# dordanino12/unet-convlstm

Measured on AMD Instinct MI355X. Metric: training frames/sec, Moving-MNIST 64x64 seq-20, higher is better.
Workload: dtype bf16; 1 GPU; TemporalUNetDualView(base_ch=64, use_skip_lstm=True) train step, 64x64 seq-20, per-GPU batch 32, AdamW+clip; global_batch=32, seq_len=20, parallelism=dp1

## Files before the change

### include/uclstm.h

```cpp
#ifndef UCLSTM_H
#define UCLSTM_H

#include <stdint.h>

#ifdef __cplusplus
extern "C" {
#endif

#define UCLSTM_ABI_VERSION 16

#define UCLSTM_OK            0
#define UCLSTM_E_BADARG     -1
#define UCLSTM_E_LAUNCH     -2
#define UCLSTM_E_NODEVICE   -3

#define UCLSTM_ACT_TYPE_BF16 0
#define UCLSTM_ACT_TYPE_F16  1


typedef struct {
    const void* ptr;
    int32_t C;
    int32_t Hs, Ws;
    int32_t offY, offX;
// ... 416 lines not shown
int32_t uclstm_head3x3_bwd_ordered(const void* a, const float* w, const float* dy, void* da, float* partials, float* dw, float* db,
                                   int32_t accumulate, int64_t n_img, int32_t H, int32_t W, int32_t Cp, int32_t C, int32_t Co,
                                   int32_t act_type, void* stream);

int32_t uclstm_maxpool3s2_bwd(const void* a, const void* dp, const void* dskip, void* da, int32_t n_img, int32_t H, int32_t W,
                              int32_t Cp, void* stream);
int64_t uclstm_bn_add_relu_bwd_rows(int64_t pixels);
int32_t uclstm_bn_add_relu_bwd_reduce(const void* z, const float* scale, const float* shift, const float* mean, const float* rstd,
                                      const void* r, const float* rscale, const float* rshift, const float* rmean,
                                      const float* rrstd, const void* da, float* partials, float* sums, float* rsums,
                                      int64_t pixels, int32_t Cp, void* stream);
int32_t uclstm_bn_add_relu_bwd_apply(const void* z, const float* scale, const float* shift, const float* mean, const float* rstd,
                                     const float* sums, const void* r, const float* rscale, const float* rshift,
                                     const float* rmean, const float* rrstd, const float* rsums, const void* da, void* dz,
                                     void* dr, int64_t pixels, int32_t Cp, void* stream);

#define UCLSTM_F16_TWIN(fn) __typeof__(fn) fn##_f16;
UCLSTM_F16_TWIN(uclstm_igemm_fwd)
UCLSTM_F16_TWIN(uclstm_igemm_fwd_group)
UCLSTM_F16_TWIN(uclstm_igemm_wgrad)
UCLSTM_F16_TWIN(uclstm_pack_weights)
UCLSTM_F16_TWIN(uclstm_pack_weights_batched)
UCLSTM_F16_TWIN(uclstm_bn_apply_relu)
UCLSTM_F16_TWIN(uclstm_bn_bwd_reduce)
UCLSTM_F16_TWIN(uclstm_bn_bwd_apply)
UCLSTM_F16_TWIN(uclstm_bn_apply_relu_pool)
UCLSTM_F16_TWIN(uclstm_bn_pool_bwd_reduce)
UCLSTM_F16_TWIN(uclstm_bn_pool_bwd_apply)
UCLSTM_F16_TWIN(uclstm_bn_head_fwd)
UCLSTM_F16_TWIN(uclstm_bn_head_bwd_reduce)
// ... 10 lines not shown
UCLSTM_F16_TWIN(uclstm_im2col3x3_first)
UCLSTM_F16_TWIN(uclstm_outconv_fwd)
UCLSTM_F16_TWIN(uclstm_outconv_bwd)
UCLSTM_F16_TWIN(uclstm_colsum)
UCLSTM_F16_TWIN(uclstm_attention_fwd)
UCLSTM_F16_TWIN(uclstm_attention_bwd)
#define UCLSTM_RESNET_F16_TWINS(TWIN) \
    TWIN(uclstm_im2col7x7s2_first) TWIN(uclstm_maxpool3s2_fwd) TWIN(uclstm_bn_add_relu) TWIN(uclstm_upsample2_fwd) \
    TWIN(uclstm_upsample2_bwd) TWIN(uclstm_head3x3_fwd) TWIN(uclstm_head3x3_bwd)
UCLSTM_RESNET_F16_TWINS(UCLSTM_F16_TWIN)
#define UCLSTM_RESNET_BWD_F16_TWINS(TWIN) \
    TWIN(uclstm_maxpool3s2_bwd) TWIN(uclstm_bn_add_relu_bwd_reduce) TWIN(uclstm_bn_add_relu_bwd_apply)
UCLSTM_RESNET_BWD_F16_TWINS(UCLSTM_F16_TWIN)
#define UCLSTM_TAP_GROUP_F16_TWINS(TWIN) TWIN(uclstm_igemm_fwd_group_tap)
UCLSTM_TAP_GROUP_F16_TWINS(UCLSTM_F16_TWIN)

int32_t uclstm_abi_version(void);
const char* uclstm_build_arch(void);
const char* uclstm_source_hash(void);
const char* uclstm_last_error_string(void);

#ifdef __cplusplus
}
#endif
#endif
```

### unet-convlstm_amd/_lib.py

```python
from __future__ import annotations

import ctypes as C
import os
import re

import torch

HERE = os.path.dirname(os.path.abspath(__file__))
LIB_PATH = os.environ.get("UCLSTM_LIB") or os.path.join(HERE, "libuclstm.so")
HEADER_PATH = os.path.join(HERE, "..", "include", "uclstm.h")

ABI_VERSION = 16
EPI_STORE, EPI_LSTM, EPI_ATOMIC = 0, 1, 2
NMODE_IDENTITY, NMODE_LSTM, NMODE_TAPMAJOR = 0, 1, 2
KMODE_IDENTITY, KMODE_GATES, KMODE_IM2COL = 0, 1, 2
ACT_TYPE_BF16, ACT_TYPE_F16 = 0, 1

_ERRORS = {-1: "bad argument (shape/alignment/null contract)", -2: "kernel launch failed", -3: "no gfx950 device"}


class UclstmError(RuntimeError):
    pass


# ... 82 lines not shown

class EvalVecDesc(C.Structure):
    _fields_ = [("y_pred", C.c_void_p), ("pred_stride_b", C.c_int64), ("pred_stride_t", C.c_int64),
                ("y", C.c_void_p), ("y_stride_b", C.c_int64), ("y_stride_t", C.c_int64),
                ("mask", C.c_void_p), ("mask_stride_b", C.c_int64), ("mask_stride_t", C.c_int64),
                ("B", C.c_int32), ("T", C.c_int32), ("Cy", C.c_int32), ("transform", C.c_int32), ("HW", C.c_int64),
                ("consts", TargetConsts * 4),
                ("hist_lo", C.c_double * 4), ("hist_hi", C.c_double * 4), ("err_lo", C.c_double * 4), ("err_hi", C.c_double * 4),
                ("dig_lo", C.c_double * 4), ("dig_w", C.c_double * 4),
                ("bins", C.c_int32), ("n_edges", C.c_int32), ("K", C.c_int32), ("dir_bins", C.c_int32),
                ("seed", C.c_uint64),
                ("w_chan", C.c_int32), ("h_chan", C.c_int32), ("w_sign", C.c_int32), ("h_sign", C.c_int32),
                ("speed_hi", C.c_double), ("epe_hi", C.c_double), ("min_speed", C.c_double),
                ("table", C.c_void_p), ("hist", C.c_void_p), ("dig_count", C.c_void_p), ("scatter", C.c_void_p),
                ("vtable", C.c_void_p), ("vhist", C.c_void_p), ("dir_hist", C.c_void_p)]


LOSS_POINT_L1, LOSS_POINT_L2, LOSS_POINT_HUBER = 0, 1, 2
VEC_MAX = 4
SELECT_MAX_SLOTS, SELECT_BINS, SELECT_SIGNED, SELECT_ABS = 8, 2048, 0, 1
SELECT_WS_COUNT, SELECT_WS_NAN, SELECT_WS_FLAGS, SELECT_WS_PREFIX, SELECT_WS_RANK, SELECT_WS_LEADER, SELECT_WS_HIST = 0, 1, 2, 8, 16, 24, 32
EXTREMES_MIN_KEY, EXTREMES_MAX_KEY, EXTREMES_NAN, EXTREMES_NONZERO, EXTREMES_COUNT, EXTREMES_WORDS = 0, 1, 2, 3, 4, 8
EVAL_ROW = 16
EVAL_VROW = 16
EVAL_NONE, EVAL_ASINH, EVAL_SIGNED_LOG = 0, 1, 2

_P, _I, _L, _F = C.c_void_p, C.c_int32, C.c_int64, C.c_float

_PROTOS = {
    "uclstm_igemm_tiles_per_group": [_I, _I, _I, _I, _I],
# ... 98 lines not shown
    "uclstm_metric_sums": [_P, _P, _P, _P, _L, _F, _F, _F, _P],
    "uclstm_metric_sums_ordered_rows": [_L],
    "uclstm_metric_sums_ordered": [_P, _P, _P, _P, _P, _I, _L, _F, _F, _F, _P],
    "uclstm_metric_sums_vec_rows": [_L, _I, _I],
    "uclstm_metric_sums_vec": [_P, _P, _P, _P, _P, _I, _L, _I, _I, _I, C.POINTER(TargetConsts), _P],
    "uclstm_eval_stats": [C.POINTER(EvalDesc), _P],
    "uclstm_eval_stats_rows": [_L, _L],
    "uclstm_eval_stats_vec": [C.POINTER(EvalVecDesc), _P],
    "uclstm_select_workspace_bytes": [],
    "uclstm_select_begin": [C.POINTER(SelectState), _P, C.POINTER(C.c_int64), C.POINTER(C.c_int32), _I, _P],
    "uclstm_select_accumulate": [C.POINTER(SelectState), _I, _P, _L, _P],
    "uclstm_select_narrow": [C.POINTER(SelectState), _I, _P],
    "uclstm_select_finish": [C.POINTER(SelectState), _P, _P, _P],
    "uclstm_dataset_extremes_begin": [_P, _P],
    "uclstm_dataset_extremes": [_P, _L, _P, _P],
    "uclstm_stream_spin": [_I, _P],
    "uclstm_abi_version": [],
    "uclstm_build_arch": [],
    "uclstm_source_hash": [],
    "uclstm_last_error_string": [],
}
_RESTYPES = {"uclstm_build_arch": C.c_char_p, "uclstm_source_hash": C.c_char_p, "uclstm_last_error_string": C.c_char_p, "uclstm_bn_bwd_reduce_rows": C.c_int64, "uclstm_bn_pool_bwd_rows": C.c_int64,
             "uclstm_eval_stats_rows": C.c_int64, "uclstm_colsum_ordered_rows": C.c_int64, "uclstm_outconv_bwd_ordered_rows": C.c_int64, "uclstm_head3x3_bwd_ordered_rows": C.c_int64,
             "uclstm_loss_fwd_ordered_rows": C.c_int64, "uclstm_sumsq_ordered_rows": C.c_int64, "uclstm_metric_sums_ordered_rows": C.c_int64, "uclstm_metric_sums_vec_rows": C.c_int64,
             "uclstm_bn_add_relu_bwd_rows": C.c_int64, "uclstm_select_workspace_bytes": C.c_int64}


F16_TWINS = ['uclstm_igemm_fwd', 'uclstm_igemm_fwd_group', 'uclstm_igemm_wgrad', 'uclstm_pack_weights', 'uclstm_pack_weights_batched', 'uclstm_bn_apply_relu', 'uclstm_bn_bwd_reduce', 'uclstm_bn_bwd_apply', 'uclstm_bn_apply_relu_pool', 'uclstm_bn_pool_bwd_reduce', 'uclstm_bn_pool_bwd_apply', 'uclstm_bn_head_fwd', 'uclstm_bn_head_bwd_reduce', 'uclstm_bn_head_bwd_apply', 'uclstm_maxpool2_fwd', 'uclstm_maxpool2_bwd', 'uclstm_lstm_bwd_pointwise', 'uclstm_lstm_fwd_pointwise', 'uclstm_lstm_fwd_pointwise_group', 'uclstm_splitk_finish', 'uclstm_nchw_to_nhwc', 'uclstm_nhwc_to_nchw', 'uclstm_nchw_grad_to_nhwc', 'uclstm_im2col3x3_first', 'uclstm_outconv_fwd', 'uclstm_outconv_bwd', 'uclstm_colsum', 'uclstm_attention_fwd', 'uclstm_attention_bwd']
RESNET_F16_TWINS = ['uclstm_im2col7x7s2_first', 'uclstm_maxpool3s2_fwd', 'uclstm_bn_add_relu', 'uclstm_upsample2_fwd', 'uclstm_upsample2_bwd',
                    'uclstm_head3x3_fwd', 'uclstm_head3x3_bwd']
RESNET_BWD_F16_TWINS = ['uclstm_maxpool3s2_bwd', 'uclstm_bn_add_relu_bwd_reduce', 'uclstm_bn_add_relu_bwd_apply']
TAP_GROUP_F16_TWINS = ['uclstm_igemm_fwd_group_tap']
_ALL_F16_TWINS = frozenset(F16_TWINS) | frozenset(RESNET_F16_TWINS) | frozenset(RESNET_BWD_F16_TWINS) | frozenset(TAP_GROUP_F16_TWINS)


def header_symbols() -> list[str]:
    with open(HEADER_PATH) as f:
        text = f.read()
    names = set(re.findall(r"\b(uclstm_[a-z0-9_]+)\s*\(", text))
    names |= {n + "_f16" for n in re.findall(r"^UCLSTM_F16_TWIN\((uclstm_[a-z0-9_]+)\)", text, re.M)}
    return sorted(names)


def _load() -> C.CDLL:
    if not os.path.exists(LIB_PATH):
        raise UclstmError(
            f"{LIB_PATH} is missing: build it with `python unet-convlstm_amd/build.py` "
            "(hipcc --offload-arch=gfx950). There is no CPU or PyTorch fallback for this package.")
# ... 55 lines not shown
```

### unet-convlstm_amd/build.py

```python
from __future__ import annotations

import hashlib
import os
import subprocess
import sys
from concurrent.futures import ThreadPoolExecutor

HERE = os.path.dirname(os.path.abspath(__file__))
CSRC = os.path.join(HERE, "csrc")
HEADER = os.path.join(HERE, "..", "include", "uclstm.h")
LIB = os.path.join(HERE, "libuclstm.so")
SOURCES = ["igemm_fwd.hip", "igemm_wgrad.hip", "pointwise.hip", "pack.hip", "loss_optim.hip", "eval_stats.hip", "augment.hip", "sprites.hip", "resnet.hip", "resnet_bwd.hip", "dataset_stats.hip"]
F16_SOURCES = ["igemm_fwd.hip", "igemm_wgrad.hip", "pointwise.hip", "pack.hip", "resnet.hip", "resnet_bwd.hip"]
FLAGS = ["--offload-arch=gfx950", "-O3", "-std=c++17", "-fPIC", "-fno-gpu-rdc", "-Wno-unused-result"]
F16_FLAGS = ["-DUCLSTM_ACT_F16", "-Wno-unused-function"]


def _hipcc() -> str:
    for c in (os.environ.get("HIPCC"), "/opt/rocm/bin/hipcc", "hipcc"):
        if c and (os.path.isabs(c) and os.path.exists(c) or not os.path.isabs(c)):
            return c
    raise RuntimeError("hipcc not found")


def _sha(parts) -> str:
    h = hashlib.sha256()
    for p in parts:
        if isinstance(p, str):
# ... 96 lines not shown
```

### unet-convlstm_amd/csrc/common.h

```cpp
#pragma once
#include <hip/hip_runtime.h>
#include <stdint.h>

#if defined(UCLSTM_ACT_F16)
#define uclstm_igemm_fwd uclstm_igemm_fwd_f16
#define uclstm_igemm_fwd_group uclstm_igemm_fwd_group_f16
#define uclstm_igemm_fwd_group_tap uclstm_igemm_fwd_group_tap_f16
#define uclstm_igemm_wgrad uclstm_igemm_wgrad_f16
#define uclstm_pack_weights uclstm_pack_weights_f16
#define uclstm_pack_weights_batched uclstm_pack_weights_batched_f16
#define uclstm_splitk_finish uclstm_splitk_finish_f16
#define uclstm_bn_apply_relu uclstm_bn_apply_relu_f16
#define uclstm_bn_bwd_reduce uclstm_bn_bwd_reduce_f16
#define uclstm_bn_bwd_apply uclstm_bn_bwd_apply_f16
#define uclstm_bn_head_fwd uclstm_bn_head_fwd_f16
#define uclstm_bn_apply_relu_pool uclstm_bn_apply_relu_pool_f16
#define uclstm_bn_pool_bwd_reduce uclstm_bn_pool_bwd_reduce_f16
#define uclstm_bn_pool_bwd_apply uclstm_bn_pool_bwd_apply_f16
#define uclstm_bn_head_bwd_reduce uclstm_bn_head_bwd_reduce_f16
#define uclstm_bn_head_bwd_apply uclstm_bn_head_bwd_apply_f16
#define uclstm_maxpool2_fwd uclstm_maxpool2_fwd_f16
#define uclstm_maxpool2_bwd uclstm_maxpool2_bwd_f16
#define uclstm_lstm_bwd_pointwise uclstm_lstm_bwd_pointwise_f16
#define uclstm_lstm_fwd_pointwise uclstm_lstm_fwd_pointwise_f16
// ... 5 lines not shown
#define uclstm_outconv_fwd uclstm_outconv_fwd_f16
#define uclstm_outconv_bwd uclstm_outconv_bwd_f16
#define uclstm_colsum uclstm_colsum_f16
#define uclstm_attention_fwd uclstm_attention_fwd_f16
#define uclstm_attention_bwd uclstm_attention_bwd_f16
#define uclstm_im2col7x7s2_first uclstm_im2col7x7s2_first_f16
#define uclstm_maxpool3s2_fwd uclstm_maxpool3s2_fwd_f16
#define uclstm_bn_add_relu uclstm_bn_add_relu_f16
#define uclstm_upsample2_fwd uclstm_upsample2_fwd_f16
#define uclstm_upsample2_bwd uclstm_upsample2_bwd_f16
#define uclstm_head3x3_fwd uclstm_head3x3_fwd_f16
#define uclstm_head3x3_bwd uclstm_head3x3_bwd_f16
#define uclstm_maxpool3s2_bwd uclstm_maxpool3s2_bwd_f16
#define uclstm_bn_add_relu_bwd_reduce uclstm_bn_add_relu_bwd_reduce_f16
#define uclstm_bn_add_relu_bwd_apply uclstm_bn_add_relu_bwd_apply_f16
#define UCLSTM_ACT_IMPL(fn) fn##_impl_f16
#else
#define UCLSTM_ACT_IMPL(fn) fn##_impl_bf16
#endif
#include "../../include/uclstm.h"

#if defined(UCLSTM_ACT_F16)
typedef _Float16 act16;
typedef __attribute__((ext_vector_type(8))) _Float16 act16x8;
typedef __attribute__((ext_vector_type(4))) _Float16 act16x4;
#define UCLSTM_MFMA_16x16x32 __builtin_amdgcn_mfma_f32_16x16x32_f16
#else
typedef __bf16 act16;
typedef __attribute__((ext_vector_type(8))) __bf16 act16x8;
typedef __attribute__((ext_vector_type(4))) __bf16 act16x4;
// ... 85 lines not shown
```

### unet-convlstm_amd/modules.py

```python
from __future__ import annotations

from typing import List, Optional, Sequence, Tuple

import torch
import torch.nn as nn

from . import ops
from ._lib import UclstmError

Tensor = torch.Tensor


def _need_grad(*ts) -> bool:
    return torch.is_grad_enabled() and any(t is not None and t.requires_grad for t in ts)


class ConvLSTMCell(nn.Module):

    def __init__(self, input_dim, hidden_dim, kernel_size=3, bias=True):
        super().__init__()
        if kernel_size % 2 == 0 or not 1 <= kernel_size <= 7:
            raise UclstmError("ConvLSTMCell: kernel_size must be odd and <= 7")
        padding = kernel_size // 2
        self.input_dim = input_dim
# ... 100 lines not shown
                _DEFERRED_COUNTERS.append((bn.num_batches_tracked, groups))
            else:
                bn.num_batches_tracked += groups
        return a

    def forward_nhwc(self, x0: Tensor, x1: Optional[Tensor] = None, c_valid=None, off=(0, 0), groups: int = 1,
                     im2col: bool = False, head=None, pool: bool = False):
        conv0, bn0, conv1, bn1 = self.net[0], self.net[1], self.net[3], self.net[4]
        if c_valid is None:
            c_valid = (conv0.in_channels,)
        a = self._stage(conv0, bn0, x0, x1, c_valid, off, groups, im2col)
        return self._stage(conv1, bn1, a, None, (conv0.out_channels,), (0, 0), groups, head=head, pool=pool)

    def first_layer_nhwc(self, x: Tensor, time_major: bool, groups: int, pool: bool = False):
        cin = self.net[0].in_channels
        if 9 * cin <= 64 and not x.requires_grad:
            return self.forward_nhwc(ops.im2col_first(x.contiguous().float(), time_major), None, (cin,), (0, 0), groups, im2col=True,
                                     pool=pool)
        if time_major:
            B, T = x.shape[0], x.shape[1]
            x = x.transpose(0, 1).reshape(B * T, *x.shape[2:])
        return self.forward_nhwc(ops.ToNHWC.apply(x.contiguous().float()), None, (cin,), (0, 0), groups, pool=pool)

    def forward(self, x):
        a = self.first_layer_nhwc(x, False, 1)
        ops.join_forward_side(a.device)
        return ops.FromNHWC.apply(a, self.net[3].out_channels)


class Down(nn.Module):
# ... 240 lines not shown
```

### unet-convlstm_amd/ops.py

```python
from __future__ import annotations

import ctypes as C
import heapq
import itertools
import os
from typing import List, Optional, Sequence, Tuple

import torch

from . import _lib as L

BF16 = torch.bfloat16
F16 = torch.float16
F32 = torch.float32
ACT = (BF16, F16)

_COMPUTE_DTYPE = BF16


def set_compute_dtype(dtype) -> None:
    global _COMPUTE_DTYPE
    if dtype not in ACT:
        raise L.UclstmError(f"compute dtype must be torch.bfloat16 or torch.float16, got {dtype}")
    _COMPUTE_DTYPE = dtype
# ... 1425 lines not shown

    @staticmethod
    def backward(ctx, da, dp=None):
        x0, x1, weight, z, par, gamma, beta, bias, head_w, head_b = ctx.saved_tensors
        c_valid, off, _, _, im2col, _, _, _ = ctx.cfg
        dz, sums, d_head_w, d_head_b = ConvBNReLU._bn_backward(ctx, z, par, head_w, head_b, da, dp)
        dbias, dgamma, dbeta = ConvBNReLU._param_grads(ctx, dz, sums, gamma, beta, bias)
        dweight = dx0 = dx1 = None
        if ctx.needs_input_grad[2]:
            dweight = conv_wgrad(weight, conv_geometry(x0, x1, weight, c_valid, off, im2col_pack_desc if im2col else None), dz)
        if ctx.needs_input_grad[0] and not im2col:
            dx0 = conv3x3_dgrad(dz, weight, x0, c_valid[0])
        if x1 is not None and ctx.needs_input_grad[1]:
            dx1 = conv3x3_dgrad(dz, weight, x1, c_valid[1], c_valid[0] * 9, -off[0], -off[1])
        return dx0, dx1, dweight, dbias, dgamma, dbeta, None, None, None, None, None, None, None, None, None, d_head_w, d_head_b, None


def _maxpool2_fwd(a: torch.Tensor) -> torch.Tensor:
    _dev(a, ACT, "activation")
    N, H, W, Cp = a.shape
    p = torch.empty((N, H // 2, W // 2, Cp), dtype=a.dtype, device=a.device)
    L.check(_k(a).uclstm_maxpool2_fwd(_p(a), _p(p), N, H, W, Cp, _stream()), "maxpool2_fwd")
    return p


def _maxpool2_bwd(a: torch.Tensor, dp: torch.Tensor, dskip: Optional[torch.Tensor]) -> torch.Tensor:
    N, H, W, Cp = a.shape
    odd = bool(H % 2 or W % 2)
    da = torch.zeros_like(a) if odd else torch.empty_like(a)
    add = dskip.contiguous() if (dskip is not None and not odd) else None
# ... 632 lines not shown
```

Measured before the change: 21130 frames/s.

## Add fused direct first-layer conv+BN+ReLU kernels with recompute-based backward

Adds a new first_stage kernel file that computes the tiny first 3x3 conv directly from the fp32 NCHW input with MFMA, fused with BN statistics and the BN+ReLU apply. The pre-activation z is recomputed instead of being stored. The backward pass likewise recomputes z on the fly to do the BN-backward reduction, and fuses the BN-backward apply with the weight-gradient reduction. The aim is to drop the NCHW->NHWC transpose, the im2col buffer and z materialisation, and several separate passes over full-resolution activations. The cost is redundant conv recompute (three times per step) and a bias gradient that is returned as zeros, on the reasoning that BN cancels it.

```diff
diff --git a/include/uclstm.h b/include/uclstm.h
--- a/include/uclstm.h
+++ b/include/uclstm.h
@@ -454,6 +454,26 @@
                                      const float* sums, const void* r, const float* rscale, const float* rshift,
                                      const float* rmean, const float* rrstd, const float* rsums, const void* da, void* dz,
                                      void* dr, int64_t pixels, int32_t Cp, void* stream);
+
+typedef struct {
+    const float* x;
+    const void* wp;
+    const float* bias;
+    int32_t n_img, C, H, W;
+    int32_t inner;
+    int32_t groups;
+    int64_t inner_stride, outer_stride;
+    int32_t Cop, Ktot;
+} uclstm_first_desc;
+int32_t uclstm_first_stats(const uclstm_first_desc* d, float* stats, void* stream);
+int32_t uclstm_first_apply(const uclstm_first_desc* d, const float* scale, const float* shift, void* a, void* stream);
+int32_t uclstm_first_z(const uclstm_first_desc* d, void* z, void* stream);
+int32_t uclstm_first_bwd_reduce(const uclstm_first_desc* d, const void* da, const float* scale, const float* shift, const float* mean,
+                                const float* rstd, float* partials, float* sums, void* stream);
+int64_t uclstm_first_wgrad_rows(int64_t pixels, int64_t pixels_per_group);
+int32_t uclstm_first_bwd_apply_wgrad(const uclstm_first_desc* d, const void* da, const float* scale, const float* shift, const float* mean,
+                                     const float* rstd, const float* sums, float* partials, float* dw, int32_t Co, int32_t accumulate,
+                                     void* stream);
 
 #define UCLSTM_F16_TWIN(fn) __typeof__(fn) fn##_f16;
 UCLSTM_F16_TWIN(uclstm_igemm_fwd)
@@ -494,6 +514,9 @@
 UCLSTM_RESNET_BWD_F16_TWINS(UCLSTM_F16_TWIN)
 #define UCLSTM_TAP_GROUP_F16_TWINS(TWIN) TWIN(uclstm_igemm_fwd_group_tap)
 UCLSTM_TAP_GROUP_F16_TWINS(UCLSTM_F16_TWIN)
+#define UCLSTM_FIRST_STAGE_F16_TWINS(TWIN) \
+    TWIN(uclstm_first_stats) TWIN(uclstm_first_apply) TWIN(uclstm_first_z) TWIN(uclstm_first_bwd_reduce) TWIN(uclstm_first_bwd_apply_wgrad)
+UCLSTM_FIRST_STAGE_F16_TWINS(UCLSTM_F16_TWIN)
 
 int32_t uclstm_abi_version(void);
 const char* uclstm_build_arch(void);
diff --git a/unet-convlstm_amd/_lib.py b/unet-convlstm_amd/_lib.py
--- a/unet-convlstm_amd/_lib.py
+++ b/unet-convlstm_amd/_lib.py
@@ -120,6 +120,14 @@
                 ("speed_hi", C.c_double), ("epe_hi", C.c_double), ("min_speed", C.c_double),
                 ("table", C.c_void_p), ("hist", C.c_void_p), ("dig_count", C.c_void_p), ("scatter", C.c_void_p),
                 ("vtable", C.c_void_p), ("vhist", C.c_void_p), ("dir_hist", C.c_void_p)]
+
+
+class FirstDesc(C.Structure):
+    _fields_ = [("x", C.c_void_p), ("wp", C.c_void_p), ("bias", C.c_void_p),
+                ("n_img", C.c_int32), ("C", C.c_int32), ("H", C.c_int32), ("W", C.c_int32),
+                ("inner", C.c_int32), ("groups", C.c_int32),
+                ("inner_stride", C.c_int64), ("outer_stride", C.c_int64),
+                ("Cop", C.c_int32), ("Ktot", C.c_int32)]
 
 
 LOSS_POINT_L1, LOSS_POINT_L2, LOSS_POINT_HUBER = 0, 1, 2
@@ -248,6 +256,12 @@
     "uclstm_select_finish": [C.POINTER(SelectState), _P, _P, _P],
     "uclstm_dataset_extremes_begin": [_P, _P],
     "uclstm_dataset_extremes": [_P, _L, _P, _P],
+    "uclstm_first_stats": [C.POINTER(FirstDesc), _P, _P],
+    "uclstm_first_apply": [C.POINTER(FirstDesc), _P, _P, _P, _P],
+    "uclstm_first_z": [C.POINTER(FirstDesc), _P, _P],
+    "uclstm_first_bwd_reduce": [C.POINTER(FirstDesc), _P, _P, _P, _P, _P, _P, _P, _P],
+    "uclstm_first_wgrad_rows": [_L, _L],
+    "uclstm_first_bwd_apply_wgrad": [C.POINTER(FirstDesc), _P, _P, _P, _P, _P, _P, _P, _P, _I, _I, _P],
     "uclstm_stream_spin": [_I, _P],
     "uclstm_abi_version": [],
     "uclstm_build_arch": [],
@@ -257,7 +271,7 @@
 _RESTYPES = {"uclstm_build_arch": C.c_char_p, "uclstm_source_hash": C.c_char_p, "uclstm_last_error_string": C.c_char_p, "uclstm_bn_bwd_reduce_rows": C.c_int64, "uclstm_bn_pool_bwd_rows": C.c_int64,
              "uclstm_eval_stats_rows": C.c_int64, "uclstm_colsum_ordered_rows": C.c_int64, "uclstm_outconv_bwd_ordered_rows": C.c_int64, "uclstm_head3x3_bwd_ordered_rows": C.c_int64,
              "uclstm_loss_fwd_ordered_rows": C.c_int64, "uclstm_sumsq_ordered_rows": C.c_int64, "uclstm_metric_sums_ordered_rows": C.c_int64, "uclstm_metric_sums_vec_rows": C.c_int64,
-             "uclstm_bn_add_relu_bwd_rows": C.c_int64, "uclstm_select_workspace_bytes": C.c_int64}
+             "uclstm_bn_add_relu_bwd_rows": C.c_int64, "uclstm_select_workspace_bytes": C.c_int64, "uclstm_first_wgrad_rows": C.c_int64}
 
 
 F16_TWINS = ['uclstm_igemm_fwd', 'uclstm_igemm_fwd_group', 'uclstm_igemm_wgrad', 'uclstm_pack_weights', 'uclstm_pack_weights_batched', 'uclstm_bn_apply_relu', 'uclstm_bn_bwd_reduce', 'uclstm_bn_bwd_apply', 'uclstm_bn_apply_relu_pool', 'uclstm_bn_pool_bwd_reduce', 'uclstm_bn_pool_bwd_apply', 'uclstm_bn_head_fwd', 'uclstm_bn_head_bwd_reduce', 'uclstm_bn_head_bwd_apply', 'uclstm_maxpool2_fwd', 'uclstm_maxpool2_bwd', 'uclstm_lstm_bwd_pointwise', 'uclstm_lstm_fwd_pointwise', 'uclstm_lstm_fwd_pointwise_group', 'uclstm_splitk_finish', 'uclstm_nchw_to_nhwc', 'uclstm_nhwc_to_nchw', 'uclstm_nchw_grad_to_nhwc', 'uclstm_im2col3x3_first', 'uclstm_outconv_fwd', 'uclstm_outconv_bwd', 'uclstm_colsum', 'uclstm_attention_fwd', 'uclstm_attention_bwd']
@@ -265,7 +279,9 @@
                     'uclstm_head3x3_fwd', 'uclstm_head3x3_bwd']
 RESNET_BWD_F16_TWINS = ['uclstm_maxpool3s2_bwd', 'uclstm_bn_add_relu_bwd_reduce', 'uclstm_bn_add_relu_bwd_apply']
 TAP_GROUP_F16_TWINS = ['uclstm_igemm_fwd_group_tap']
-_ALL_F16_TWINS = frozenset(F16_TWINS) | frozenset(RESNET_F16_TWINS) | frozenset(RESNET_BWD_F16_TWINS) | frozenset(TAP_GROUP_F16_TWINS)
+FIRST_STAGE_F16_TWINS = ['uclstm_first_stats', 'uclstm_first_apply', 'uclstm_first_z', 'uclstm_first_bwd_reduce', 'uclstm_first_bwd_apply_wgrad']
+_ALL_F16_TWINS = (frozenset(F16_TWINS) | frozenset(RESNET_F16_TWINS) | frozenset(RESNET_BWD_F16_TWINS) | frozenset(TAP_GROUP_F16_TWINS)
+                  | frozenset(FIRST_STAGE_F16_TWINS))
 
 
 def header_symbols() -> list[str]:
diff --git a/unet-convlstm_amd/build.py b/unet-convlstm_amd/build.py
--- a/unet-convlstm_amd/build.py
+++ b/unet-convlstm_amd/build.py
@@ -10,8 +10,8 @@
 CSRC = os.path.join(HERE, "csrc")
 HEADER = os.path.join(HERE, "..", "include", "uclstm.h")
 LIB = os.path.join(HERE, "libuclstm.so")
-SOURCES = ["igemm_fwd.hip", "igemm_wgrad.hip", "pointwise.hip", "pack.hip", "loss_optim.hip", "eval_stats.hip", "augment.hip", "sprites.hip", "resnet.hip", "resnet_bwd.hip", "dataset_stats.hip"]
-F16_SOURCES = ["igemm_fwd.hip", "igemm_wgrad.hip", "pointwise.hip", "pack.hip", "resnet.hip", "resnet_bwd.hip"]
+SOURCES = ["igemm_fwd.hip", "igemm_wgrad.hip", "pointwise.hip", "pack.hip", "loss_optim.hip", "eval_stats.hip", "augment.hip", "sprites.hip", "resnet.hip", "resnet_bwd.hip", "dataset_stats.hip", "first_stage.hip"]
+F16_SOURCES = ["igemm_fwd.hip", "igemm_wgrad.hip", "pointwise.hip", "pack.hip", "resnet.hip", "resnet_bwd.hip", "first_stage.hip"]
 FLAGS = ["--offload-arch=gfx950", "-O3", "-std=c++17", "-fPIC", "-fno-gpu-rdc", "-Wno-unused-result"]
 F16_FLAGS = ["-DUCLSTM_ACT_F16", "-Wno-unused-function"]
 
diff --git a/unet-convlstm_amd/csrc/common.h b/unet-convlstm_amd/csrc/common.h
--- a/unet-convlstm_amd/csrc/common.h
+++ b/unet-convlstm_amd/csrc/common.h
@@ -43,6 +43,11 @@
 #define uclstm_maxpool3s2_bwd uclstm_maxpool3s2_bwd_f16
 #define uclstm_bn_add_relu_bwd_reduce uclstm_bn_add_relu_bwd_reduce_f16
 #define uclstm_bn_add_relu_bwd_apply uclstm_bn_add_relu_bwd_apply_f16
+#define uclstm_first_stats uclstm_first_stats_f16
+#define uclstm_first_apply uclstm_first_apply_f16
+#define uclstm_first_z uclstm_first_z_f16
+#define uclstm_first_bwd_reduce uclstm_first_bwd_reduce_f16
+#define uclstm_first_bwd_apply_wgrad uclstm_first_bwd_apply_wgrad_f16
 #define UCLSTM_ACT_IMPL(fn) fn##_impl_f16
 #else
 #define UCLSTM_ACT_IMPL(fn) fn##_impl_bf16
diff --git a/unet-convlstm_amd/csrc/first_stage.hip b/unet-convlstm_amd/csrc/first_stage.hip
--- /dev/null
+++ b/unet-convlstm_amd/csrc/first_stage.hip
@@ -0,0 +1,508 @@
+#include "common.h"
+#include <algorithm>
+
+namespace {
+
+constexpr int FS_NT = 256;
+constexpr int FS_TILE = 256;
+constexpr int FS_CHUNK = 128;
+constexpr int FS_TPITCH = FS_CHUNK * 2 + 16;
+
+struct FirstGeom {
+    const float* x;
+    const act16* wp;
+    const float* bias;
+    int C, H, W, HW;
+    int Cop, Ktot, na;
+    FastDiv dHW, dW, dinner;
+    int64_t inner_stride, outer_stride;
+};
+
+struct FirstLane {
+    int koff[8];
+    int kdy[8], kdx[8];
+    act16x8 wf[4];
+    float bs[4][4];
+};
+
+__device__ __forceinline__ void first_lane_init(const FirstGeom& G, FirstLane& L) {
+    const int lane = threadIdx.x & 63, l15 = lane & 15, lq = lane >> 4;
+#pragma unroll
+    for (int i = 0; i < 8; ++i) {
+        const int k = lq * 8 + i;
+        const int tap = k / G.C, c = k - tap * G.C;
+        const bool ok = tap < 9;
+        const int dy = tap / 3 - 1, dx = tap % 3 - 1;
+        L.kdy[i] = ok ? dy : 0x40000000;
+        L.kdx[i] = ok ? dx : 0;
+        L.koff[i] = ok ? c * G.HW + dy * G.W + dx : 0;
+    }
+#pragma unroll
+    for (int a = 0; a < 4; ++a) {
+        const int row = a * 16 + l15;
+        Pack16 w;
+        w.u = row < G.Cop ? *(const uint4*)(G.wp + (long)row * G.Ktot + lq * 8) : make_uint4(0u, 0u, 0u, 0u);
+        L.wf[a] = w.v;
+#pragma unroll
+        for (int r = 0; r < 4; ++r) {
+            const int n = a * 16 + lq * 4 + r;
+            L.bs[a][r] = (G.bias && n < G.Cop) ? G.bias[n] : 0.f;
+        }
+    }
+}
+
+__device__ __forceinline__ void first_zfrag(const FirstGeom& G, const FirstLane& L, int64_t p, bool pok, f32x4 (&acc)[4], act16x8& xf) {
+    const uint32_t m = pok ? (uint32_t)p : 0u;
+    const uint32_t img = fdiv(m, G.dHW);
+    const int rem = (int)(m - img * (uint32_t)G.HW);
+    const int y = (int)fdiv((uint32_t)rem, G.dW);
+    const int xx = rem - y * G.W;
+    const uint32_t o = fdiv(img, G.dinner);
+    const uint32_t in = img - o * G.dinner.d;
+    const float* src = G.x + (int64_t)in * G.outer_stride + (int64_t)o * G.inner_stride;
+    float t[8];
+#pragma unroll
+    for (int i = 0; i < 8; ++i) {
+        const bool ok = pok && (unsigned)(y + L.kdy[i]) < (unsigned)G.H && (unsigned)(xx + L.kdx[i]) < (unsigned)G.W;
+        const float v = src[ok ? rem + L.koff[i] : 0];
+        t[i] = ok ? v : 0.f;
+    }
+    Pack16 pk;
+#pragma unroll
+    for (int i = 0; i < 8; ++i) pk.e[i] = f32_to_act(t[i]);
+    xf = pk.v;
+#pragma unroll
+    for (int a = 0; a < 4; ++a)
+        if (a < G.na) acc[a] = UCLSTM_MFMA_16x16x32(L.wf[a], xf, (f32x4){0.f, 0.f, 0.f, 0.f}, 0, 0, 0);
+}
+
+__device__ __forceinline__ void first_zstage(const FirstGeom& G, const FirstLane& L, const f32x4 (&acc)[4], unsigned char* Zs, int pitch, int row) {
+    const int lq = (threadIdx.x & 63) >> 4;
+#pragma unroll
+    for (int a = 0; a < 4; ++a) {
+        const int col = a * 16 + lq * 4;
+        if (a < G.na && col < G.Cop) {
+            Pack8 o;
+#pragma unroll
+            for (int r = 0; r < 4; ++r) o.e[r] = f32_to_act(acc[a][r] + L.bs[a][r]);
+            *(uint2*)(Zs + row * pitch + col * 2) = o.u;
+        }
+    }
+}
+
+__device__ __forceinline__ void first_ztile(const FirstGeom& G, const FirstLane& L, unsigned char* Zs, int pitch, int64_t pbeg, int nrows) {
+    const int l15 = threadIdx.x & 15, wave = threadIdx.x >> 6;
+    for (int f = wave; f * 16 < nrows; f += FS_NT / 64) {
+        f32x4 acc[4];
+        act16x8 xf;
+        const int row = f * 16 + l15;
+        first_zfrag(G, L, pbeg + row, row < nrows, acc, xf);
+        first_zstage(G, L, acc, Zs, pitch, row);
+    }
+}
+
+__device__ __forceinline__ void fs_unpack8(const uint4 u, float (&f)[8]) {
+    Pack16 p;
+    p.u = u;
+#pragma unroll
+    for (int i = 0; i < 8; ++i) f[i] = act_to_f32(p.e[i]);
+}
+__device__ __forceinline__ uint4 fs_pack8(const float (&f)[8]) {
+    Pack16 p;
+#pragma unroll
+    for (int i = 0; i < 8; ++i) p.e[i] = f32_to_act(f[i]);
+    return p.u;
+}
+__device__ __forceinline__ void fs_load8f(const float* p, float (&f)[8]) {
+    const float4 a = *(const float4*)p, b = *(const float4*)(p + 4);
+    f[0] = a.x; f[1] = a.y; f[2] = a.z; f[3] = a.w; f[4] = b.x; f[5] = b.y; f[6] = b.z; f[7] = b.w;
+}
+
+__global__ __launch_bounds__(FS_NT) void first_stats_kernel(const FirstGeom G, float* __restrict__ stats, int64_t ppg, int tpg) {
+    extern __shared__ __attribute__((aligned(16))) unsigned char smem[];
+    const int pitch = G.Cop * 2 + 16;
+    FirstLane L;
+    first_lane_init(G, L);
+    const int g = blockIdx.x / tpg, tile = blockIdx.x - g * tpg;
+    const int64_t pbeg = (int64_t)g * ppg + (int64_t)tile * FS_TILE;
+    const int rows_valid = (int)min((int64_t)FS_TILE, (int64_t)(g + 1) * ppg - pbeg);
+    first_ztile(G, L, smem, pitch, pbeg, rows_valid);
+    __syncthreads();
+    const int j = threadIdx.x & 7;
+    for (int col = threadIdx.x >> 3; col < G.Cop; col += FS_NT / 8) {
+        float s1 = 0.f, s2 = 0.f;
+        for (int r = j; r < rows_valid; r += 8) {
+            const float v = act_to_f32(*(const act16*)(smem + r * pitch + col * 2));
+            s1 += v;
+            s2 += v * v;
+        }
+        s1 += __shfl_xor(s1, 4); s2 += __shfl_xor(s2, 4);
+        s1 += __shfl_xor(s1, 1); s2 += __shfl_xor(s2, 1);
+        s1 += __shfl_xor(s1, 2); s2 += __shfl_xor(s2, 2);
+        if (j == 0) {
+            float* sp = stats + ((long)blockIdx.x * G.Cop + col) * 2;
+            sp[0] = s1;
+            sp[1] = s2;
+        }
+    }
+}
+
+template <bool RAW>
+__global__ __launch_bounds__(FS_NT) void first_apply_kernel(const FirstGeom G, const float* __restrict__ scale, const float* __restrict__ shift,
+                                                            uint4* __restrict__ out, int64_t pixels, FastDiv dppg, int ntiles) {
+    extern __shared__ __attribute__((aligned(16))) unsigned char smem[];
+    const int pitch = G.Cop * 2 + 16, cpc = G.Cop / 8;
+    FirstLane L;
+    first_lane_init(G, L);
+    for (int tile = blockIdx.x; tile < ntiles; tile += gridDim.x) {
+        const int64_t pbeg = (int64_t)tile * FS_TILE;
+        const int rows_valid = (int)min((int64_t)FS_TILE, pixels - pbeg);
+        first_ztile(G, L, smem, pitch, pbeg, rows_valid);
+        __syncthreads();
+        for (int q = threadIdx.x; q < rows_valid * cpc; q += FS_NT) {
+            const int r = q / cpc, cc = q - r * cpc;
+            const int64_t pix = pbeg + r;
+            const uint4 zq = *(const uint4*)(smem + r * pitch + cc * 16);
+            if (RAW) {
+                out[pix * cpc + cc] = zq;
+            } else {
+                const uint32_t g = fdiv((uint32_t)pix, dppg);
+                const long so = (long)g * G.Cop + cc * 8;
+                float v[8], sc[8], sh[8];
+                fs_unpack8(zq, v);
+                fs_load8f(scale + so, sc);
+                fs_load8f(shift + so, sh);
+#pragma unroll
+                for (int i = 0; i < 8; ++i) v[i] = fmaxf(v[i] * sc[i] + sh[i], 0.f);
+                out[pix * cpc + cc] = fs_pack8(v);
+            }
+        }
+        __syncthreads();
+    }
+}
+
+__global__ __launch_bounds__(FS_NT) void first_bwd_reduce_kernel(const FirstGeom G, const uint4* __restrict__ da, const float* __restrict__ scale,
+                                                                 const float* __restrict__ shift, const float* __restrict__ mean,
+                                                                 const float* __restrict__ rstd, float* __restrict__ partials, int64_t ppg,
+                                                                 int rows, int blocks_per_group) {
+    extern __shared__ __attribute__((aligned(16))) unsigned char smem[];
+    float* red = (float*)smem;
+    const int Cp = G.Cop, cpc = Cp / 8, pitch = Cp * 2 + 16;
+    FirstLane L;
+    first_lane_init(G, L);
+    const int g = blockIdx.x / blocks_per_group;
+    const int bi = blockIdx.x - g * blocks_per_group;
+    const int64_t gbeg = (int64_t)g * ppg, gend = gbeg + ppg;
+    const int sweep = 4 * rows;
+    const int cc = threadIdx.x % cpc, prow = threadIdx.x / cpc;
+    const bool act = (int)threadIdx.x < rows * cpc;
+    float s1[8] = {0, 0, 0, 0, 0, 0, 0, 0}, s2[8] = {0, 0, 0, 0, 0, 0, 0, 0};
+    float sc[8], sh[8], mu[8];
+    const long so = (long)g * Cp + cc * 8;
+    fs_load8f(scale + so, sc);
+    fs_load8f(shift + so, sh);
+    fs_load8f(mean + so, mu);
+    for (int64_t s0 = gbeg + (int64_t)bi * sweep; s0 < gend; s0 += (int64_t)sweep * blocks_per_group) {
+        uint4 gq[4];
+        bool ok[4];
+#pragma unroll
+        for (int u = 0; u < 4; ++u) {
+            const int64_t p = s0 + prow + u * rows;
+            ok[u] = act && p < gend;
+            gq[u] = ok[u] ? da[p * cpc + cc] : make_uint4(0u, 0u, 0u, 0u);
+        }
+        first_ztile(G, L, smem, pitch, s0, (int)min((int64_t)sweep, gend - s0));
+        __syncthreads();
+#pragma unroll
+        for (int u = 0; u < 4; ++u) {
+            if (ok[u]) {
+                float zv[8], gv[8];
+                fs_unpack8(*(const uint4*)(smem + (prow + u * rows) * pitch + cc * 16), zv);
+                fs_unpack8(gq[u], gv);
+#pragma unroll
+                for (int i = 0; i < 8; ++i) {
+                    const float g0 = (zv[i] * sc[i] + sh[i] > 0.f) ? gv[i] : 0.f;
+                    s1[i] += g0;
+                    s2[i] = fmaf(g0, zv[i] - mu[i], s2[i]);
+                }
+            }
+        }
+        __syncthreads();
+    }
+    const int width = cpc * 16;
+    if (act) {
+        float rs[8];
+        fs_load8f(rstd + so, rs);
+#pragma unroll
+        for (int i = 0; i < 8; ++i) s2[i] *= rs[i];
+        float* r = red + prow * width + cc * 16;
+#pragma unroll
+        for (int i = 0; i < 8; ++i) {
+            r[i * 2] = s1[i];
+            r[i * 2 + 1] = s2[i];
+        }
+    }
+    __syncthreads();
+    for (int j = threadIdx.x; j < width; j += FS_NT) {
+        float t = 0.f;
+        for (int r = 0; r < rows; ++r) t += red[r * width + j];
+        partials[((long)blockIdx.x * Cp + (j >> 1)) * 2 + (j & 1)] = t;
+    }
+}
+
+__global__ __launch_bounds__(256) void first_bwd_sum_kernel(const float* __restrict__ partials, float* __restrict__ sums, int blocks_per_group,
+                                                            int Cp) {
+    __shared__ double red[8][32];
+    const int g = blockIdx.y;
+    const int e = blockIdx.x * 32 + (threadIdx.x & 31);
+    const int lane = threadIdx.x >> 5;
+    double t = 0.0;
+    if (e < Cp * 2)
+        for (int b = lane; b < blocks_per_group; b += 8) t += (double)partials[((long)(g * blocks_per_group + b) * Cp) * 2 + e];
+    red[lane][threadIdx.x & 31] = t;
+    __syncthreads();
+    if (lane == 0 && e < Cp * 2) {
+        double s = 0.0;
+#pragma unroll
+        for (int k = 0; k < 8; ++k) s += red[k][threadIdx.x];
+        sums[(long)g * Cp * 2 + e] = (float)s;
+    }
+}
+
+__global__ __launch_bounds__(FS_NT) void first_bwd_wgrad_kernel(const FirstGeom G, const unsigned char* __restrict__ da, const float* __restrict__ scale,
+                                                                const float* __restrict__ shift, const float* __restrict__ mean,
+                                                                const float* __restrict__ rstd, const float* __restrict__ sums,
+                                                                float* __restrict__ partials, int64_t ppg, int blocks_per_group,
+                                                                int64_t pix_per_block, float inv_n, int Co) {
+    extern __shared__ __attribute__((aligned(16))) unsigned char smem[];
+    unsigned char* DzT = smem;
+    unsigned char* XT = smem + 64 * FS_TPITCH;
+    const int lane = threadIdx.x & 63, l15 = lane & 15, lq = lane >> 4, wave = threadIdx.x >> 6;
+    const int Cp = G.Cop, K9 = 9 * G.C;
+    FirstLane L;
+    first_lane_init(G, L);
+    const int g = blockIdx.x / blocks_per_group;
+    const int bi = blockIdx.x - g * blocks_per_group;
+    const int64_t p0 = (int64_t)g * ppg + (int64_t)bi * pix_per_block;
+    const int64_t p1 = min((int64_t)(g + 1) * ppg, p0 + pix_per_block);
+    float sc[4][4], sh[4][4], k1[4][4], k0[4][4];
+#pragma unroll
+    for (int a = 0; a < 4; ++a)
+#pragma unroll
+        for (int r = 0; r < 4; ++r) {
+            const int n = a * 16 + lq * 4 + r;
+            sc[a][r] = sh[a][r] = k1[a][r] = k0[a][r] = 0.f;
+            if (n < Cp) {
+                const long so = (long)g * Cp + n;
+                sc[a][r] = scale[so];
+                sh[a][r] = shift[so];
+                k1[a][r] = -sc[a][r] * rstd[so] * sums[so * 2 + 1] * inv_n;
+                k0[a][r] = -sc[a][r] * sums[so * 2] * inv_n - k1[a][r] * mean[so];
+            }
+        }
+    for (int q = threadIdx.x; q < 64 * FS_TPITCH / 16; q += FS_NT) ((uint4*)DzT)[q] = make_uint4(0u, 0u, 0u, 0u);
+    __syncthreads();
+    f32x4 dacc[4][2];
+#pragma unroll
+    for (int a = 0; a < 4; ++a) dacc[a][0] = dacc[a][1] = (f32x4){0.f, 0.f, 0.f, 0.f};
+    const int nst0 = (lq & 1) ? 16 + (lq - 1) * 4 : lq * 4;
+    for (int64_t c0 = p0; c0 < p1; c0 += FS_CHUNK) {
+        const int64_t wbeg = c0 + wave * 32;
+#pragma unroll
+        for (int f = 0; f < 2; ++f) {
+            const int64_t p = wbeg + f * 16 + l15;
+            const bool pok = p < p1;
+            uint4 gq[2];
+#pragma unroll
+            for (int h = 0; h < 2; ++h)
+                gq[h] = (pok && h * 32 + nst0 < Cp) ? *(const uint4*)(da + (p * Cp + h * 32 + nst0) * 2) : make_uint4(0u, 0u, 0u, 0u);
+            f32x4 acc[4];
+            act16x8 xf;
+            first_zfrag(G, L, p, pok, acc, xf);
+            const int px = wave * 32 + f * 16 + l15;
+            Pack16 xk;
+            xk.v = xf;
+#pragma unroll
+            for (int i = 0; i < 8; ++i) *(act16*)(XT + (lq * 8 + i) * FS_TPITCH + px * 2) = xk.e[i];
+#pragma unroll
+            for (int h = 0; h < 2; ++h) {
+                const auto q0 = __builtin_amdgcn_permlane16_swap(gq[h].x, gq[h].z, false, false);
+                const auto q1 = __builtin_amdgcn_permlane16_swap(gq[h].y, gq[h].w, false, false);
+#pragma unroll
+                for (int a2 = 0; a2 < 2; ++a2) {
+                    const int a = 2 * h + a2;
+                    Pack8 gv;
+                    gv.u = make_uint2(q0[a2], q1[a2]);
+                    if (a < G.na && a * 16 + lq * 4 < Cp) {
+#pragma unroll
+                        for (int r = 0; r < 4; ++r) {
+                            const float zv = act_to_f32(f32_to_act(acc[a][r] + L.bs[a][r]));
+                            const float gg = act_to_f32(gv.e[r]);
+                            const float o = ((zv * sc[a][r] + sh[a][r] > 0.f) ? sc[a][r] * gg : 0.f) + k1[a][r] * zv + k0[a][r];
+                            *(act16*)(DzT + (a * 16 + lq * 4 + r) * FS_TPITCH + px * 2) = f32_to_act(pok ? o : 0.f);
+                        }
+                    }
+                }
+            }
+        }
+        __syncthreads();
+        {
+            const int off = (wave * 32 + lq * 8) * 2;
+            const act16x8 b0 = *(const act16x8*)(XT + l15 * FS_TPITCH + off);
+            const act16x8 b1 = *(const act16x8*)(XT + (16 + l15) * FS_TPITCH + off);
+#pragma unroll
+            for (int a = 0; a < 4; ++a) {
+                if (a < G.na) {
+                    const act16x8 af = *(const act16x8*)(DzT + (a * 16 + l15) * FS_TPITCH + off);
+                    dacc[a][0] = UCLSTM_MFMA_16x16x32(af, b0, dacc[a][0], 0, 0, 0);
+                    if (K9 > 16) dacc[a][1] = UCLSTM_MFMA_16x16x32(af, b1, dacc[a][1], 0, 0, 0);
+                }
+            }
+        }
+        __syncthreads();
+    }
+    float* red = (float*)smem;
+#pragma unroll
+    for (int a = 0; a < 4; ++a)
+#pragma unroll
+        for (int kt = 0; kt < 2; ++kt)
+#pragma unroll
+            for (int r = 0; r < 4; ++r) red[(wave * 64 + a * 16 + lq * 4 + r) * 32 + kt * 16 + l15] = dacc[a][kt][r];
+    __syncthreads();
+    const int E = Co * K9;
+    for (int e = threadIdx.x; e < E; e += FS_NT) {
+        const int co = e / K9, rem = e - co * K9;
+        const int ci = rem / 9, tap = rem - ci * 9;
+        const int k = tap * G.C + ci;
+        float t = red[(0 * 64 + co) * 32 + k];
+#pragma unroll
+        for (int w = 1; w < 4; ++w) t += red[(w * 64 + co) * 32 + k];
+        partials[(long)blockIdx.x * E + e] = t;
+    }
+}
+
+__global__ __launch_bounds__(256) void first_wgrad_finish_kernel(const float* __restrict__ partials, int rows, int E, float* __restrict__ dw,
+                                                                 int accumulate) {
+    __shared__ double red[32][8];
+    const int e = blockIdx.x * 8 + (threadIdx.x & 7);
+    const int lane = threadIdx.x >> 3;
+    double t = 0.0;
+    if (e < E) {
+#pragma unroll 8
+        for (int b = lane; b < rows; b += 32) t += (double)partials[(long)b * E + e];
+    }
+    red[lane][threadIdx.x & 7] = t;
+    __syncthreads();
+    if (lane == 0 && e < E) {
+        double s = 0.0;
+#pragma unroll
+        for (int k = 0; k < 32; ++k) s += red[k][threadIdx.x];
+        dw[e] = accumulate ? dw[e] + (float)s : (float)s;
+    }
+}
+
+bool fs_aligned16(const void* p) { return p && ((uintptr_t)p % 16) == 0; }
+
+bool first_geom(const uclstm_first_desc* d, FirstGeom& G) {
+    if (!d || !d->x || !fs_aligned16(d->wp) || (d->bias && ((uintptr_t)d->bias % 4)) || d->n_img <= 0 || d->C <= 0 || 9 * d->C > 32 || d->H <= 0 ||
+        d->W <= 0 || d->inner <= 0 || (d->n_img % d->inner) || d->groups <= 0 || (d->n_img % d->groups) || d->Cop <= 0 || (d->Cop % 8) ||
+        d->Cop > 64 || d->Ktot < 32 || (d->Ktot % 8) || d->inner_stride < 0 || d->outer_stride < 0)
+        return false;
+    if ((int64_t)d->n_img * d->H * d->W >= ((int64_t)1 << 31) || (int64_t)d->C * d->H * d->W >= ((int64_t)1 << 30)) return false;
+    G.x = d->x;
+    G.wp = (const act16*)d->wp;
+    G.bias = d->bias;
+    G.C = d->C; G.H = d->H; G.W = d->W; G.HW = d->H * d->W;
+    G.Cop = d->Cop; G.Ktot = d->Ktot; G.na = (d->Cop + 15) / 16;
+    G.dHW = make_fastdiv((uint32_t)G.HW);
+    G.dW = make_fastdiv((uint32_t)d->W);
+    G.dinner = make_fastdiv((uint32_t)d->inner);
+    G.inner_stride = d->inner_stride;
+    G.outer_stride = d->outer_stride;
+    return true;
+}
+
+inline int first_wgrad_bpg(int64_t ppg, int groups) {
+    int64_t bpg = (ppg + FS_CHUNK - 1) / FS_CHUNK;
+    const int64_t cap = std::max(1, 1024 / groups);
+    return (int)std::min(bpg, cap);
+}
+
+}
+
+extern "C" int32_t uclstm_first_stats(const uclstm_first_desc* d, float* stats, void* stream) {
+    FirstGeom G;
+    if (!first_geom(d, G) || !stats) return UCLSTM_E_BADARG;
+    const int64_t ppg = (int64_t)(d->n_img / d->groups) * G.HW;
+    const int tpg = (int)((ppg + FS_TILE - 1) / FS_TILE);
+    UCLSTM_LAUNCH(first_stats_kernel, dim3((unsigned)(d->groups * tpg)), dim3(FS_NT), (size_t)FS_TILE * (G.Cop * 2 + 16), (hipStream_t)stream, G,
+                  stats, ppg, tpg);
+    return UCLSTM_OK;
+}
+
+static int32_t first_apply_launch(const uclstm_first_desc* d, const float* scale, const float* shift, void* out, bool raw, void* stream) {
+    FirstGeom G;
+    if (!first_geom(d, G) || !fs_aligned16(out) || (!raw && (!fs_aligned16(scale) || !fs_aligned16(shift)))) return UCLSTM_E_BADARG;
+    const int64_t pixels = (int64_t)d->n_img * G.HW, ppg = pixels / d->groups;
+    const int ntiles = (int)((pixels + FS_TILE - 1) / FS_TILE);
+    const int grid = std::min(ntiles, 256 * 8);
+    const size_t lds = (size_t)FS_TILE * (G.Cop * 2 + 16);
+    if (raw)
+        UCLSTM_LAUNCH(first_apply_kernel<true>, dim3(grid), dim3(FS_NT), lds, (hipStream_t)stream, G, scale, shift, (uint4*)out, pixels,
+                      make_fastdiv((uint32_t)ppg), ntiles);
+    else
+        UCLSTM_LAUNCH(first_apply_kernel<false>, dim3(grid), dim3(FS_NT), lds, (hipStream_t)stream, G, scale, shift, (uint4*)out, pixels,
+                      make_fastdiv((uint32_t)ppg), ntiles);
+    return UCLSTM_OK;
+}
+
+extern "C" int32_t uclstm_first_apply(const uclstm_first_desc* d, const float* scale, const float* shift, void* a, void* stream) {
+    return first_apply_launch(d, scale, shift, a, false, stream);
+}
+
+extern "C" int32_t uclstm_first_z(const uclstm_first_desc* d, void* z, void* stream) {
+    return first_apply_launch(d, nullptr, nullptr, z, true, stream);
+}
+
+extern "C" int32_t uclstm_first_bwd_reduce(const uclstm_first_desc* d, const void* da, const float* scale, const float* shift, const float* mean,
+                                           const float* rstd, float* partials, float* sums, void* stream) {
+    FirstGeom G;
+    if (!first_geom(d, G) || !fs_aligned16(da) || !fs_aligned16(scale) || !fs_aligned16(shift) || !fs_aligned16(mean) || !fs_aligned16(rstd) ||
+        !partials || !sums)
+        return UCLSTM_E_BADARG;
+    const int64_t pixels = (int64_t)d->n_img * G.HW, ppg = pixels / d->groups;
+    const int bpg = (int)(uclstm_bn_bwd_reduce_rows(pixels, ppg) / d->groups);
+    const int cpc = G.Cop / 8, rows = FS_NT / cpc;
+    const int srows = (4 * rows + 15) / 16 * 16;
+    const size_t lds = std::max((size_t)srows * (G.Cop * 2 + 16), (size_t)rows * cpc * 16 * sizeof(float));
+    UCLSTM_LAUNCH(first_bwd_reduce_kernel, dim3((unsigned)(d->groups * bpg)), dim3(FS_NT), lds, (hipStream_t)stream, G, (const uint4*)da, scale,
+                  shift, mean, rstd, partials, ppg, rows, bpg);
+    UCLSTM_LAUNCH(first_bwd_sum_kernel, dim3((G.Cop * 2 + 31) / 32, d->groups), dim3(256), 0, (hipStream_t)stream, partials, sums, bpg, G.Cop);
+    return UCLSTM_OK;
+}
+
+#ifndef UCLSTM_ACT_F16
+extern "C" int64_t uclstm_first_wgrad_rows(int64_t pixels, int64_t pixels_per_group) {
+    if (pixels <= 0 || pixels_per_group <= 0 || (pixels % pixels_per_group)) return UCLSTM_E_BADARG;
+    const int groups = (int)(pixels / pixels_per_group);
+    return (int64_t)groups * first_wgrad_bpg(pixels_per_group, groups);
+}
+#endif
+
+extern "C" int32_t uclstm_first_bwd_apply_wgrad(const uclstm_first_desc* d, const void* da, const float* scale, const float* shift,
+                                                const float* mean, const float* rstd, const float* sums, float* partials, float* dw,
+                                                int32_t Co, int32_t accumulate, void* stream) {
+    FirstGeom G;
+    if (!first_geom(d, G) || !fs_aligned16(da) || !scale || !shift || !mean || !rstd || !sums || !partials || !dw || Co <= 0 || Co > d->Cop)
+        return UCLSTM_E_BADARG;
+    const int64_t pixels = (int64_t)d->n_img * G.HW, ppg = pixels / d->groups;
+    const int bpg = first_wgrad_bpg(ppg, d->groups);
+    const int64_t ppb = (ppg + bpg - 1) / bpg;
+    const int rows = d->groups * bpg, E = Co * 9 * G.C;
+    const size_t lds = std::max((size_t)96 * FS_TPITCH, (size_t)4 * 64 * 32 * sizeof(float));
+    UCLSTM_LAUNCH(first_bwd_wgrad_kernel, dim3((unsigned)rows), dim3(FS_NT), lds, (hipStream_t)stream, G, (const unsigned char*)da, scale, shift,
+                  mean, rstd, sums, partials, ppg, bpg, ppb, (float)(1.0 / (double)ppg), (int)Co);
+    UCLSTM_LAUNCH(first_wgrad_finish_kernel, dim3((unsigned)((E + 7) / 8)), dim3(256), 0, (hipStream_t)stream, partials, rows, E, dw,
+                  (int)accumulate);
+    return UCLSTM_OK;
+}
diff --git a/unet-convlstm_amd/modules.py b/unet-convlstm_amd/modules.py
--- a/unet-convlstm_amd/modules.py
+++ b/unet-convlstm_amd/modules.py
@@ -138,6 +138,17 @@
 
     def first_layer_nhwc(self, x: Tensor, time_major: bool, groups: int, pool: bool = False):
         cin = self.net[0].in_channels
+        conv0, bn0 = self.net[0], self.net[1]
+        training, mom = bn_mode(bn0, self.training)
+        if ops.first_direct_ok(x, conv0.weight, training):
+            a = ops.FirstConvBNReLU.apply(x.contiguous(), conv0.weight, conv0.bias, bn0.weight, bn0.bias, bn0.running_mean, bn0.running_var,
+                                          bool(time_major), groups, mom, bn0.eps)
+            if bn0.num_batches_tracked is not None:
+                if _DEFERRED_COUNTERS is not None:
+                    _DEFERRED_COUNTERS.append((bn0.num_batches_tracked, groups))
+                else:
+                    bn0.num_batches_tracked += groups
+            return self._stage(self.net[3], self.net[4], a, None, (conv0.out_channels,), (0, 0), groups, pool=pool)
         if 9 * cin <= 64 and not x.requires_grad:
             return self.forward_nhwc(ops.im2col_first(x.contiguous().float(), time_major), None, (cin,), (0, 0), groups, im2col=True,
                                      pool=pool)
diff --git a/unet-convlstm_amd/ops.py b/unet-convlstm_amd/ops.py
--- a/unet-convlstm_amd/ops.py
+++ b/unet-convlstm_amd/ops.py
@@ -1463,6 +1463,116 @@
         if x1 is not None and ctx.needs_input_grad[1]:
             dx1 = conv3x3_dgrad(dz, weight, x1, c_valid[1], c_valid[0] * 9, -off[0], -off[1])
         return dx0, dx1, dweight, dbias, dgamma, dbeta, None, None, None, None, None, None, None, None, None, d_head_w, d_head_b, None
+
+
+def first_direct_mode() -> str:
+    v = os.environ.get("UCLSTM_FIRST_DIRECT", "1").strip().lower()
+    return v if v in ("0", "fwd") else "1"
+
+
+def first_direct_ok(x: torch.Tensor, weight: torch.Tensor, training: bool) -> bool:
+    return (first_direct_mode() != "0" and training and isinstance(x, torch.Tensor) and x.dtype == F32 and not x.requires_grad
+            and x.dim() in (4, 5) and weight.dim() == 4 and weight.shape[2] == weight.shape[3] == 3 and 9 * weight.shape[1] <= 32
+            and cpad(weight.shape[0]) <= 64 and x.numel() // x.shape[-3] < (1 << 31))
+
+
+def _first_geometry(x: torch.Tensor, time_major: bool):
+    if time_major:
+        B, T, Cc, H, W = x.shape
+        return B * T, Cc, H, W, B, Cc * H * W, T * Cc * H * W
+    n_img, Cc, H, W = x.shape
+    return n_img, Cc, H, W, n_img, 0, Cc * H * W
+
+
+def first_desc(x: torch.Tensor, time_major: bool, wp: torch.Tensor, bp: Optional[torch.Tensor], groups: int, Cop: int) -> L.FirstDesc:
+    n_img, Cc, H, W, inner, inner_stride, outer_stride = _first_geometry(x, time_major)
+    d = L.FirstDesc()
+    d.x, d.wp, d.bias = x.data_ptr(), wp.data_ptr(), (bp.data_ptr() if bp is not None else None)
+    d.n_img, d.C, d.H, d.W, d.inner, d.groups = n_img, Cc, H, W, inner, groups
+    d.inner_stride, d.outer_stride = inner_stride, outer_stride
+    d.Cop, d.Ktot = Cop, wp.numel() // Cop
+    return d
+
+
+def _log_first(kind: str) -> None:
+    if LAUNCH_LOG is not None:
+        LAUNCH_LOG.append(("first", kind))
+
+
+class FirstConvBNReLU(_GradAwareFunction):
+
+    @staticmethod
+    def forward(ctx, x, weight, bias, gamma, beta, running_mean, running_var, time_major, groups, momentum, eps):
+        _dev(x, F32, "input")
+        n_img, Cc, H, W, _, _, _ = _first_geometry(x, time_major)
+        Co, Cop, dev, dt = weight.shape[0], cpad(weight.shape[0]), x.device, _COMPUTE_DTYPE
+        pd = im2col_pack_desc(Co, Cc, cpad(9 * Cc))
+        wp = pack_weights(pd, weight, 0, dt)
+        bp = pack_bias(pd, bias) if bias is not None else None
+        K = L.kernels(dt)
+        d = first_desc(x, time_major, wp, bp, groups, Cop)
+        stats = torch.empty((groups, L.lib.uclstm_igemm_tiles_per_group(n_img, H, W, groups, Cop), Cop, 2), dtype=F32, device=dev)
+        _log_first("first_stats")
+        _timed_hbm("first_stats", 4.0 * x.numel(), lambda: L.check(K.uclstm_first_stats(C.byref(d), _p(stats), _stream()), "first_stats"))
+        par, sync = _bn_forward_stats(stats, n_img, H, W, groups, Co, gamma, beta, running_mean, running_var, momentum, eps, "plain")
+        a = torch.empty((n_img, H, W, Cop), dtype=dt, device=dev)
+        _log_first("first_apply")
+        _timed_hbm("first_apply", 2.0 * a.numel() + 4.0 * x.numel(),
+                   lambda: L.check(K.uclstm_first_apply(C.byref(d), _p(par[0]), _p(par[1]), _p(a), _stream()), "first_apply"))
+        ctx.save_for_backward(x, weight, wp, bp, par, gamma, beta, bias)
+        ctx.cfg = (bool(time_major), groups, Co, first_direct_mode())
+        ctx.sync_bn = sync
+        if _will_backward(ctx):
+            note_use(weight, gamma, beta, bias)
+        return a
+
+    @staticmethod
+    def backward(ctx, da):
+        x, weight, wp, bp, par, gamma, beta, bias = ctx.saved_tensors
+        time_major, groups, Co, mode = ctx.cfg
+        da = da.contiguous()
+        (n_img, H, W, Cop), dev = da.shape, da.device
+        pixels, ppg = n_img * H * W, (n_img // groups) * H * W
+        K = _k(da)
+        d = first_desc(x, time_major, wp, bp, groups, Cop)
+        pq = (_p(par[0]), _p(par[1]), _p(par[2]), _p(par[3]))
+        need_w, need_b, need_gamma, need_beta = ctx.needs_input_grad[1:5]
+        dweight = None
+        if mode == "fwd":
+            z = torch.empty_like(da)
+            _log_first("first_z")
+            _timed_hbm("first_z", 2.0 * z.numel() + 4.0 * x.numel(), lambda: L.check(K.uclstm_first_z(C.byref(d), _p(z), _stream()), "first_z"))
+            dz, sums = bn_relu_backward(z, par, da, groups, True, ctx.sync_bn, want_dz=need_w)
+            if need_w:
+                xg = im2col_first(x, time_major)
+                dweight = conv_wgrad(weight, conv_geometry(xg, None, weight, (weight.shape[1],), (0, 0), im2col_pack_desc), dz)
+        else:
+            sums = torch.empty((groups, Cop, 2), dtype=F32, device=dev)
+            partials = torch.empty((int(L.lib.uclstm_bn_bwd_reduce_rows(pixels, ppg)), Cop, 2), dtype=F32, device=dev)
+            _log_first("first_bwd_reduce")
+            _timed_hbm("first_bwd_reduce", 2.0 * da.numel() + 4.0 * x.numel(),
+                       lambda: L.check(K.uclstm_first_bwd_reduce(C.byref(d), _p(da), *pq, _p(partials), _p(sums), _stream()), "first_bwd_reduce"))
+            if need_w:
+                sums_dz = sums if ctx.sync_bn is None else _bn_bwd_sums_over_ranks(sums, ctx.sync_bn, "plain")
+                g = direct_grad(weight)
+                dw = g if g is not None else torch.empty(weight.shape, dtype=F32, device=dev)
+                rows = torch.empty((int(L.lib.uclstm_first_wgrad_rows(pixels, ppg)), weight.numel()), dtype=F32, device=dev)
+                _log_first("first_bwd_apply_wgrad")
+                _timed_hbm("first_bwd_apply_wgrad", 2.0 * da.numel() + 4.0 * x.numel(),
+                           lambda: L.check(K.uclstm_first_bwd_apply_wgrad(C.byref(d), _p(da), *pq, _p(sums_dz), _p(rows), _p(dw), Co,
+                                                                          1 if g is not None else 0, _stream()), "first_bwd_apply_wgrad"))
+                if g is not None:
+                    grad_written(weight)
+                else:
+                    dweight = dw
+        dgamma, dbeta, direct = bn_param_grads(need_gamma, need_beta, gamma, beta, sums, Co)
+        dbias = None
+        if need_b and bias is not None:
+            if direct and direct_grad(bias) is not None:
+                grad_written(bias)
+            else:
+                dbias = torch.zeros((Co,), dtype=F32, device=dev)
+        return None, dweight, dbias, dgamma, dbeta, None, None, None, None, None, None
 
 
 def _maxpool2_fwd(a: torch.Tensor) -> torch.Tensor:
```

After: 21280 frames/s (median of 6 runs). About the same (+0.7%).
